# joesound212985/Deepfake-Detection-using-CLIP-Based-SigLIP-2-Vision-Transformers

Hardware: AMD Instinct MI355X
Metric: images/sec (train fwd+bwd) SigLIP-2-so400m@384 bf16 (higher is better)
Workload: dtype bf16; 1 GPU; so400m-patch14-384 encoder+pool-head train fwd+bwd, 384x384, per-GPU batch 128, seeded random weights; global_batch=128, parallelism=dp1

## Files before the change

### deepfake-detection-using-clip-based-siglip-2-vision-transformers_amd/csrc/epilogue.hip.h

```cpp
#pragma once
#include <type_traits>

#include "common.hip.h"
#include "kernels.h"

namespace sgl {

template <int NV>
__device__ __forceinline__ void epi_res_f32(float* v, const float* bias, const float* r, float* dst) {
#pragma unroll
  for (int j = 0; j < NV; ++j) v[j] = r[j] + (v[j] + bias[j]);
  Vec<float, NV>::st_nt(dst, v);
}
template <typename TOut, int NV>
__device__ __forceinline__ void epi_bias_gelu(const EpiParams& p, float* v, const float* bias, TOut* dst_u, TOut* dst_act) {
  float a[NV];
  if (p.out && p.gelu_grad_form) {
#pragma unroll
    for (int j = 0; j < NV; ++j) gelu_tanh_both(v[j] + bias[j], a[j], v[j]);
  } else {
#pragma unroll
    for (int j = 0; j < NV; ++j) {
      v[j] += bias[j];
      a[j] = gelu_tanh(v[j]);
    }
  }
  if (p.out) Vec<TOut, NV>::st_nt(dst_u, v);
  Vec<TOut, NV>::st_nt(dst_act, a);
}
__device__ __forceinline__ void qkv_split_row(int row, int tokens, int& b, int& n) {
  b = (int)((float)row * __builtin_amdgcn_rcpf((float)tokens));
  n = row - b * tokens;
  if (n < 0) { b -= 1; n += tokens; }
  else if (n >= tokens) { b += 1; n -= tokens; }
}
template <typename TOut, int NV>
__device__ __forceinline__ void epi_qkv(float* v, const float* bias, TOut* dst, int pad_chunks) {
#pragma unroll
  for (int j = 0; j < NV; ++j) v[j] += bias[j];
  Vec<TOut, NV>::st_nt(dst, v);
  if (pad_chunks) {
    float z[NV];
#pragma unroll
    for (int j = 0; j < NV; ++j) z[j] = 0.f;
    for (int k = 1; k <= pad_chunks; ++k) Vec<TOut, NV>::st_nt(dst + k * NV, z);
  }
}
template <typename TOut, int NV>
__device__ __forceinline__ void epi_gelu_bwd(const EpiParams& p, float* v, const float* u, TOut* dst) {
  if (p.gelu_grad_form) {
#pragma unroll
    for (int j = 0; j < NV; ++j) v[j] *= u[j];
  } else {
#pragma unroll
    for (int j = 0; j < NV; ++j) v[j] *= gelu_tanh_grad(u[j]);
  }
  Vec<TOut, NV>::st_nt(dst, v);
}

__device__ __forceinline__ void lds_barrier() {
  asm volatile("s_waitcnt lgkmcnt(0)" ::: "memory");
  __builtin_amdgcn_s_barrier();
  asm volatile("" ::: "memory");
}

template <int NT, int BN, int NV>
__device__ __forceinline__ void epi_colsum_fold(float* ct, const float (&csum)[NV], int t, int m0, int n0, int N,
                                                const EpiParams& p) {
  constexpr int CPR = BN / NV, GROUPS = NT / CPR;
  static_assert(NT % CPR == 0 && BN <= NT, "one fixed column set per thread, one thread per column");
  if (!p.colsum) return;
  lds_barrier();
#pragma unroll
  for (int j = 0; j < NV; ++j) ct[(t / CPR) * BN + (t % CPR) * NV + j] = csum[j];
  lds_barrier();
  if (t < BN && n0 + t < N) {
    float s = 0.f;
#pragma unroll
    for (int gI = 0; gI < GROUPS; ++gI) s += ct[gI * BN + t];
    if (p.colsum_ld > 0)
      p.colsum[(size_t)(m0 >> 7) * p.colsum_ld + n0 + t] = s;
    else
      atomicAdd(p.colsum + n0 + t, s);
  }
}

template <int EPI, typename TOut, int NV>
__device__ __forceinline__ void epi_apply(const EpiParams& p, int row, int col, int N, float* v) {
  if constexpr (EPI == EPI_STORE) {
#pragma unroll
    for (int j = 0; j < NV; ++j) v[j] *= p.alpha;
    if (p.bias) {
      float b[NV];
      Vec<float, NV>::ld(p.bias + col, b);
#pragma unroll
      for (int j = 0; j < NV; ++j) v[j] += b[j];
    }
    Vec<TOut, NV>::st_nt(reinterpret_cast<TOut*>(p.out) + (size_t)row * p.ldo + col, v);
  } else if constexpr (EPI == EPI_BIAS_GELU) {
// ... 79 lines not shown
```

### deepfake-detection-using-clip-based-siglip-2-vision-transformers_amd/csrc/gemm_bf16.hip

```cpp
#include <stdlib.h>

#include "common.hip.h"
#include "epilogue.hip.h"
#include "kernels.h"

namespace sgl {

constexpr int G_BM = 128, G_BN = 128, G_BK = 64;
constexpr int G_STAGE = (G_BM + G_BN) * G_BK * 2;
constexpr int G_CT_LD = 132;
constexpr int G_LDS = (2 * G_STAGE > G_BM * G_CT_LD * 4) ? 2 * G_STAGE : G_BM * G_CT_LD * 4;

__device__ __forceinline__ u32x4 ldg128(__amdgpu_buffer_rsrc_t r, uint32_t voff) {
  return __builtin_amdgcn_raw_buffer_load_b128(r, voff, 0, 0);
}

template <int EPI, typename TOut>
__device__ __forceinline__ void store_tile(char* smem, f32x4 (&acc)[4][4], int wr, int wc, int lane, int t, int m0,
                                           int n0, int M, int N, const EpiParams& p) {
  float* ct = reinterpret_cast<float*>(smem);
  __syncthreads();
  const int g = lane >> 4, c16 = lane & 15;
#pragma unroll
  for (int i = 0; i < 4; ++i)
// ... 197 lines not shown
  store_stage(0);
  __syncthreads();
  for (int kt = 0; kt < nk; ++kt) {
    const int cur = kt & 1;
    if (kt + 1 < nk) load_tile(kt + 1);
    const char* base = smem + cur * G_STAGE;
#pragma unroll
    for (int s = 0; s < 2; ++s) {
      const char* ba = base + s * 32 * 256 + frow;
      const char* bb = ba + OPB;
      lo_x8<TIn> af[4], bfr[4];
#pragma unroll
      for (int i = 0; i < 4; ++i) {
        const lo_x4<TIn> alo = lds_read_tr16<TIn>(ba + fa_col[i]);
        const lo_x4<TIn> ahi = lds_read_tr16<TIn>(ba + 4 * 256 + fa_col[i]);
        const lo_x4<TIn> blo = lds_read_tr16<TIn>(bb + fb_col[i]);
        const lo_x4<TIn> bhi = lds_read_tr16<TIn>(bb + 4 * 256 + fb_col[i]);
        af[i] = __builtin_shufflevector(alo, ahi, 0, 1, 2, 3, 4, 5, 6, 7);
        bfr[i] = __builtin_shufflevector(blo, bhi, 0, 1, 2, 3, 4, 5, 6, 7);
      }
#pragma unroll
      for (int i = 0; i < 4; ++i)
#pragma unroll
        for (int j = 0; j < 4; ++j)
          acc[i][j] = mfma_16x16x32(af[i], bfr[j], acc[i][j]);
    }
    if (kt + 1 < nk) store_stage(cur ^ 1);
    __syncthreads();
  }
  EpiParams pq = p;
  if (p.split_stride) pq.out = reinterpret_cast<float*>(p.out) + (size_t)blockIdx.y * p.split_stride;
  store_tile<EPI_F32, float>(smem, acc, wr, wc, lane, t, n1_0, n2_0, N1, N2, pq);
}

template <int EPI, typename TOut, typename TIn>
static hipError_t launch_nt(const TIn* A, int lda, const TIn* B, int ldb, int M, int N, int K, const EpiParams& p,
                            hipStream_t s) {
  const hipError_t e = set_max_dynamic_lds_once<&gemm_nt_kernel<EPI, TOut, TIn>>(G_LDS);
  if (e != hipSuccess) return e;
  const int tiles = ((M + G_BM - 1) / G_BM) * ((N + G_BN - 1) / G_BN);
  hipLaunchKernelGGL((gemm_nt_kernel<EPI, TOut, TIn>), dim3(tiles), dim3(256), G_LDS, s, A, lda, B, ldb, M, N, K, p);
  return hipGetLastError();
}

template <typename TIn>
static hipError_t gemm_nt_mfma(const void* A, int lda, const void* B, int ldb, int M, int N, int K, int epi,
                               int out_dtype, const EpiParams& p, hipStream_t s) {
  if (M == 0 || N == 0) return hipSuccess;
  if ((lda % 8) || (ldb % 8) || (K % 8) || K <= 0) return hipErrorInvalidValue;
  if (epi != EPI_F32 && (N % 8)) return hipErrorInvalidValue;
  if ((size_t)M * lda * 2 >= (1ull << 32) || (size_t)N * ldb * 2 >= (1ull << 32)) return hipErrorInvalidValue;
  if (M >= 2048 && N >= 256) {
    static const int tile_env = getenv("SGL_NT_TILE") ? atoi(getenv("SGL_NT_TILE")) : 0;
    const bool can384 = epi == EPI_STORE || epi == EPI_RES_F32;
    const bool pays384 = N % 192 == 0 && N % 256 != 0 && (epi == EPI_STORE || K >= 2048);
    const bool want384 = tile_env == 384 || (tile_env != 256 && pays384);
    if (can384 && want384) return gemm_nt384<TIn>(A, lda, B, ldb, M, N, K, epi, out_dtype, p, s);
    return gemm_nt256<TIn>(A, lda, B, ldb, M, N, K, epi, out_dtype, p, s);
  }
  return dispatch_epilogue<TIn>(epi, out_dtype, [&](auto tag) {
    using T = decltype(tag);
    return launch_nt<T::epi, typename T::out, TIn>((const TIn*)A, lda, (const TIn*)B, ldb, M, N, K, p, s);
  });
}
hipError_t gemm_nt_bf16(const void* A, int lda, const void* B, int ldb, int M, int N, int K, int epi, int out_dtype,
                        const EpiParams& p, hipStream_t s) {
  return gemm_nt_mfma<bf16>(A, lda, B, ldb, M, N, K, epi, out_dtype, p, s);
}
hipError_t gemm_nt_f16(const void* A, int lda, const void* B, int ldb, int M, int N, int K, int epi, int out_dtype,
                       const EpiParams& p, hipStream_t s) {
  return gemm_nt_mfma<f16>(A, lda, B, ldb, M, N, K, epi, out_dtype, p, s);
}

static bool tn_slabs_ok(const EpiParams& p, int N2, const float* split_ws) {
  return p.alpha == 1.0f && !p.bias && (N2 % 4 == 0) && (p.ldo % 4 == 0) &&
         ((((uintptr_t)p.out) | ((uintptr_t)split_ws)) & 15) == 0;
}

template <typename Launch>
static hipError_t tn_split_k(int Mred, int N1, int N2, int splits, const EpiParams& p_, hipStream_t s, float* split_ws,
                             size_t split_ws_bytes, Launch&& launch) {
  EpiParams p = p_;
  float* out = reinterpret_cast<float*>(p.out);
  if (splits < 1) splits = 1;
  int m_per = (Mred + splits - 1) / splits;
  m_per = ((m_per + G_BK - 1) / G_BK) * G_BK;
  splits = (Mred + m_per - 1) / m_per;
  if (splits > 1) {
    const size_t slab = (size_t)N1 * N2;
    if (split_ws && (size_t)splits * slab * sizeof(float) <= split_ws_bytes && tn_slabs_ok(p, N2, split_ws)) {
      EpiParams q = p;
      q.out = split_ws;
      q.ldo = N2;
      q.accumulate = 0;
      q.atomic = 0;
      q.split_stride = slab;
      const hipError_t e = launch(m_per, splits, q);
      if (e != hipSuccess) return e;
      return reduce_splits(split_ws, splits, slab, N1, N2, out, p.ldo, p.accumulate, s);
    }
    if (!p.accumulate) {
      const hipError_t e = hipMemset2DAsync(out, (size_t)p.ldo * sizeof(float), 0, (size_t)N2 * sizeof(float), N1, s);
      if (e != hipSuccess) return e;
    }
    p.atomic = 1;
  }
// ... 45 lines not shown
```

### deepfake-detection-using-clip-based-siglip-2-vision-transformers_amd/csrc/gemm_bf16_v2.hip

```cpp
#include <stdlib.h>
#ifdef SGL_TIMELINE
#include <stdio.h>
#include <string.h>
#endif

#include "common.hip.h"
#include "epilogue.hip.h"
#include "kernels.h"

namespace sgl {

constexpr int T_BK = 64;

template <int BM_, int BN_, int MI_, int MJ_>
struct NtTileShape {
  static constexpr int BM = BM_, BN = BN_, MI = MI_, MJ = MJ_;
  static constexpr int WM = 16 * MI, WN = 16 * MJ;
  static constexpr int NWR = BM / WM, NWC = BN / WN;
  static constexpr int OPA = BM * T_BK * 2;
  static constexpr int STAGE = (BM + BN) * T_BK * 2;
  static constexpr int LDS = 2 * STAGE;
  static constexpr int PA = BM / 128, PB = BN / 64, NI = 2 * PA + PB;
  static constexpr int CT_LD = BN + 4;
  static_assert(NWR * WM == BM && NWC * WN == BN && NWR * NWC == 8, "8 waves = 512 threads cover the tile");
  static_assert(MI % 2 == 0 && BM % 128 == 0 && BN % 64 == 0 && 64 % NWR == 0 && (64 / NWR) % 16 == 0, "halves, pieces, passes");
  static_assert(LDS <= 160 * 1024 && 64 * CT_LD * 4 <= LDS, "two stages, and the epilogue image, in 160 KiB of LDS");
};

struct NtTile256 : NtTileShape<256, 256, 8, 4> {
  static __device__ __forceinline__ int wr(int w) { return (w >> 1) & 1; }
  static __device__ __forceinline__ int wc(int w) { return (w & 1) + 2 * (w >> 2); }
  static __device__ __forceinline__ int b_row(int w, int q) {
    const int ul = 16 * w + 8 * (q & 1);
    return (ul >> 5) * 64 + (ul & 31) + 32 * (q >> 1);
  }
  static constexpr bool takes(int epi) { return true; }
};

struct NtTile384 : NtTileShape<384, 192, 6, 6> {
  static __device__ __forceinline__ int wr(int w) { return w & 3; }
  static __device__ __forceinline__ int wc(int w) { return w >> 2; }
  static __device__ __forceinline__ int b_row(int w, int q) { return 8 * (3 * w + q); }
  static constexpr bool takes(int epi) { return epi == EPI_STORE || epi == EPI_RES_F32 || epi == EPI_F32; }
};

constexpr int gcd_of(int a, int b) { return b == 0 ? a : gcd_of(b, a % b); }

template <typename G, int EPI, typename TOut>
__device__ __forceinline__ void store_tile_pp(char* smem, f32x4 (&acc)[G::MI][G::MJ], int wr, int wc, int lane, int t,
                                              int m0, int n0, int M, int N, const EpiParams& p) {
  static_assert(G::takes(EPI), "this tile geometry is not dispatched with this epilogue");
  float* ct = reinterpret_cast<float*>(smem);
  const int g = lane >> 4, c16 = lane & 15;
  constexpr int NV = (sizeof(TOut) == 4) ? 4 : 8;
  constexpr int CT_LD = G::CT_LD;
  constexpr int CPR = G::BN / NV;
  constexpr int WR_ROWS = 64 / G::NWR;
  constexpr int BLK = WR_ROWS / 16;
  constexpr int NPASS = G::BM / 64;
  constexpr int QN = (64 * CPR) / 512;
  constexpr int P = CPR / gcd_of(CPR, 512);
  static_assert(NPASS * BLK == G::MI && (64 * CPR) % 512 == 0 && (512 * P) % CPR == 0, "staging image and chunk walk");
  auto grow_of = [&](int pass, int row) { return m0 + (row / WR_ROWS) * G::WM + pass * WR_ROWS + row % WR_ROWS; };
  constexpr bool HAS_BIAS = (EPI == EPI_BIAS_GELU || EPI == EPI_RES_F32 || EPI == EPI_QKV);
  int tcol[P], gcol[P];
  bool col_ok[P];
  float bias[P][NV];
  size_t qkv_c0[P];
  int qkv_pad[P];
#pragma unroll
  for (int h = 0; h < P; ++h) {
    tcol[h] = ((t + 512 * h) % CPR) * NV;
    gcol[h] = n0 + tcol[h];
    col_ok[h] = gcol[h] < N;
#pragma unroll
    for (int j = 0; j < NV; ++j) bias[h][j] = 0.f;
    if constexpr (HAS_BIAS) {
      if (col_ok[h]) Vec<float, NV>::ld(p.bias + gcol[h], bias[h]);
    }
    qkv_c0[h] = 0;
    qkv_pad[h] = 0;
    if constexpr (EPI == EPI_QKV) {
      const int dm = p.heads * p.head_dim;
      const int which = gcol[h] / dm;
      const int hc = gcol[h] - which * dm;
      const int hd = hc / p.head_dim;
      const int d = hc - hd * p.head_dim;
      qkv_c0[h] = ((size_t)which * p.batch * p.heads + hd) * (size_t)p.tokens * p.head_dim_pad + d;
      qkv_pad[h] = (d + NV == p.head_dim) ? (p.head_dim_pad - p.head_dim) / NV : 0;
    }
  }
  float csum[NV];
#pragma unroll
  for (int j = 0; j < NV; ++j) csum[j] = 0.f;
  using PreT = u32x4;
  constexpr bool HAS_PRE = (EPI == EPI_RES_F32 || EPI == EPI_GELU_BWD);
// ... 41 lines not shown
        }
        continue;
      }
    }
#pragma unroll
    for (int q = 0; q < QN; ++q) {
      const int h = q % P;
      const int row = (t + 512 * q) / CPR;
      const int grow = grow_of(pass, row);
      if (grow < M && col_ok[h]) {
        float v[NV];
        Vec<float, NV>::ld(ct + row * CT_LD + tcol[h], v);
        if constexpr (EPI == EPI_RES_F32) {
          const f32x4 r = __builtin_bit_cast(f32x4, pre[pass & 1][q]);
          float rf[NV];
#pragma unroll
          for (int j = 0; j < NV; ++j) rf[j] = r[j];
          epi_res_f32<NV>(v, bias[h], rf, reinterpret_cast<float*>(p.out) + (size_t)grow * p.ldo + gcol[h]);
        } else if constexpr (EPI == EPI_BIAS_GELU) {
          epi_bias_gelu<TOut, NV>(p, v, bias[h], reinterpret_cast<TOut*>(p.out) + (size_t)grow * p.ldo + gcol[h],
                                  reinterpret_cast<TOut*>(p.out2) + (size_t)grow * p.ldo2 + gcol[h]);
        } else if constexpr (EPI == EPI_QKV) {
          int b, n;
          qkv_split_row(grow, p.tokens, b, n);
          epi_qkv<TOut, NV>(v, bias[h],
                            reinterpret_cast<TOut*>(p.out) + qkv_c0[h] + ((size_t)b * p.heads * p.tokens + n) * p.head_dim_pad,
                            qkv_pad[h]);
        } else if constexpr (EPI == EPI_GELU_BWD) {
          float u[NV];
          if constexpr (NV == 8) {
            const lo_x8<TOut> ub = __builtin_bit_cast(lo_x8<TOut>, pre[pass & 1][q]);
#pragma unroll
            for (int j = 0; j < NV; ++j) u[j] = (float)ub[j];
          } else {
            const f32x4 uf = __builtin_bit_cast(f32x4, pre[pass & 1][q]);
#pragma unroll
            for (int j = 0; j < NV; ++j) u[j] = uf[j];
          }
          epi_gelu_bwd<TOut, NV>(p, v, u, reinterpret_cast<TOut*>(p.out) + (size_t)grow * p.ldo + gcol[h]);
#pragma unroll
          for (int j = 0; j < NV; ++j) csum[j] += v[j];
        } else {
          epi_apply<EPI, TOut, NV>(p, grow, gcol[h], N, v);
        }
      }
    }
  }
  if constexpr (EPI == EPI_GELU_BWD) {
    static_assert(P == 1, "the bias-gradient fold needs one column set per thread");
    epi_colsum_fold<512, G::BN, NV>(ct, csum, t, m0, n0, N, p);
  }
}

__device__ __forceinline__ int unit_of_block(int bid, int per) { return (bid & 7) * per + (bid >> 3); }

__device__ __forceinline__ void tile_of_unit(int u, int tiles_m, int tiles_n, int& tile_m, int& tile_n, int bh = 8) {
  const int band = u / (bh * tiles_n);
  const int rows = (tiles_m - band * bh < bh) ? tiles_m - band * bh : bh;
  const int r = u - band * bh * tiles_n;
  tile_n = r / rows;
  tile_m = band * bh + (r - tile_n * rows);
}

__device__ __forceinline__ bool tile_of_local(int xcd, int v, int tiles_m, int tiles_n, int cgw, int& tm, int& tn) {
  const int r_lo = (xcd * tiles_m) >> 3, r_hi = ((xcd + 1) * tiles_m) >> 3;
  const int R = r_hi - r_lo;
  if (v >= R * tiles_n) return false;
  const int full = R * cgw;
  const int g = v / full, rem = v - g * full;
  const int w = (tiles_n - g * cgw < cgw) ? tiles_n - g * cgw : cgw;
  const int r = rem / w;
  tm = r_lo + r;
  tn = g * cgw + (rem - r * w);
  return true;
}

__device__ __forceinline__ void pp_dma16(u32x4 desc, uint32_t lds_addr, uint32_t voff) {
  asm volatile("s_mov_b32 m0, %0\n\ts_nop 0\n\tbuffer_load_dwordx4 %1, %2, 0 offen lds"
               :: "s"(lds_addr), "v"(voff), "s"(desc) : "memory");
}
__device__ __forceinline__ u32x4 pp_desc(const void* base, uint32_t bytes) {
  const uint64_t q = (uint64_t)base;
  u32x4 d = {(uint32_t)q, (uint32_t)(q >> 32) & 0xffffu, bytes, 0x00020000u};
  return d;
}
__device__ __forceinline__ u32x4 pp_desc_sgpr(u32x4 d) {
  return u32x4{(uint32_t)__builtin_amdgcn_readfirstlane((int)d[0]), (uint32_t)__builtin_amdgcn_readfirstlane((int)d[1]),
               (uint32_t)__builtin_amdgcn_readfirstlane((int)d[2]), (uint32_t)__builtin_amdgcn_readfirstlane((int)d[3])};
}
template <int NI>
__device__ __forceinline__ void pp_end_read() {
  asm volatile("s_waitcnt vmcnt(%0) lgkmcnt(0)" :: "n"(NI) : "memory");
  __builtin_amdgcn_sched_barrier(0);
  __builtin_amdgcn_s_barrier();
  __builtin_amdgcn_sched_barrier(0);
}
#define SGL_PP_END_MFMA()                 \
  do {                                    \
    __builtin_amdgcn_sched_barrier(0);    \
    __builtin_amdgcn_s_barrier();         \
    __builtin_amdgcn_sched_barrier(0);    \
  } while (0)

#ifdef SGL_TIMELINE
__device__ unsigned long long g_nt6_tl[4];
__device__ unsigned long long g_tn6_tl[12];
#define SGL_TL_STAMP(v) const unsigned long long v = __builtin_readcyclecounter()
#else
#define SGL_TL_STAMP(v)
#endif

template <typename G, int EPI, typename TOut, typename TIn>
__global__ __launch_bounds__(512, 2) void gemm_nt6_kernel(const TIn* __restrict__ A, int lda,
                                                          const TIn* __restrict__ B, int ldb, int M, int N, int K,
                                                          int tiles_m, int tiles_n, int band_h, EpiParams p) {
  extern __shared__ __attribute__((aligned(16))) char smem[];
  SGL_TL_STAMP(tl0);
  const int ntiles = tiles_m * tiles_n;
  int tile_m, tile_n;
  if (band_h < 0) {
    if (!tile_of_local(blockIdx.x & 7, blockIdx.x >> 3, tiles_m, tiles_n, -band_h, tile_m, tile_n)) return;
  } else {
    const int unit = unit_of_block(blockIdx.x, (ntiles + 7) >> 3);
    if (unit >= ntiles) return;
    tile_of_unit(unit, tiles_m, tiles_n, tile_m, tile_n, band_h);
  }
  constexpr int MI = G::MI, MJ = G::MJ, HI = MI / 2, PA = G::PA, PB = G::PB, NI = G::NI;
  const int t = threadIdx.x, lane = t & 63;
  const int w = __builtin_amdgcn_readfirstlane(t >> 6);
  const int wr = G::wr(w), wc = G::wc(w), grp = w >> 2;
  const int m0 = tile_m * G::BM, n0 = tile_n * G::BN;
  const int rows_a = (M - m0 < G::BM) ? M - m0 : G::BM;
  const int rows_b = (N - n0 < G::BN) ? N - n0 : G::BN;
  const u32x4 da = pp_desc(A + (size_t)m0 * lda, (uint32_t)(((size_t)(rows_a - 1) * lda + K) * 2));
  const u32x4 db = pp_desc(B + (size_t)n0 * ldb, (uint32_t)(((size_t)(rows_b - 1) * ldb + K) * 2));
  const uint32_t lds0 = (uint32_t)(size_t)((SGL_LDS char*)smem);

  enum { U_A0 = 0, U_B = 1, U_A1 = 2 };
  constexpr int PMAX = PA > PB ? PA : PB;
  const int drow = lane >> 3, dchunk = (lane & 7) ^ drow;
  uint32_t voff[3][PMAX], ldst[3][PMAX];
#pragma unroll
  for (int u = 0; u < 3; ++u)
#pragma unroll
    for (int q = 0; q < (u == U_B ? PB : PA); ++q) {
      const bool isA = u != U_B;
      constexpr int ppw = G::WM / 16;
      const int piece = PA * w + q;
      const int r0 = isA ? G::WM * (piece / ppw) + 8 * (piece % ppw) + (u == U_A1 ? G::WM / 2 : 0) : G::b_row(w, q);
      const int row = r0 + drow;
      voff[u][q] = (row < (isA ? rows_a : rows_b)) ? (uint32_t)(row * (isA ? lda : ldb) + dchunk * 8) * 2u : SGL_OOB;
      ldst[u][q] = lds0 + (isA ? 0 : G::OPA) + (uint32_t)r0 * 128u;
    }
  const int nk = (K + T_BK - 1) / T_BK;
  auto issue = [&](int u, int kt) {
    const int k0 = kt * T_BK;
    const bool kok = (kt < nk) && (k0 + dchunk * 8 < K);
    const uint32_t sb = (uint32_t)((kt & 1) * G::STAGE);
#pragma unroll
    for (int q = 0; q < (u == U_B ? PB : PA); ++q)
      pp_dma16(u == U_B ? db : da, ldst[u][q] + sb, (kok && voff[u][q] != SGL_OOB) ? voff[u][q] + (uint32_t)k0 * 2u : SGL_OOB);
  };

  const int frow = lane & 15, fg = lane >> 4, fsw = frow & 7;
  const uint32_t fa_base = (uint32_t)((wr * G::WM + frow) * 128);
  const uint32_t fb_base = (uint32_t)(G::OPA + (wc * G::WN + frow) * 128);
  const uint32_t c0 = (uint32_t)(((0 + fg) ^ fsw) << 4), c1 = (uint32_t)(((4 + fg) ^ fsw) << 4);
  const bool active = (n0 + wc * G::WN < N) && (m0 + wr * G::WM < M);

  f32x4 acc[MI][MJ];
#pragma unroll
  for (int i = 0; i < MI; ++i)
#pragma unroll
    for (int j = 0; j < MJ; ++j) acc[i][j] = f32x4{0.f, 0.f, 0.f, 0.f};

  issue(U_A0, 0); issue(U_B, 0); issue(U_A1, 0);
  issue(U_A0, 1); issue(U_B, 1);
  pp_end_read<NI>();
  if (grp == 1) SGL_PP_END_MFMA();

  lo_x8<TIn> fa[2 * HI], fb[2 * MJ];
  auto mfma_slot = [&](int i0) {
    if (active) {
      __builtin_amdgcn_s_setprio(1);
#pragma unroll
      for (int h = 0; h < 2; ++h)
#pragma unroll
        for (int i = 0; i < HI; ++i)
#pragma unroll
          for (int j = 0; j < MJ; ++j)
            acc[i0 + i][j] = mfma_16x16x32(fa[HI * h + i], fb[MJ * h + j], acc[i0 + i][j]);
      __builtin_amdgcn_s_setprio(0);
    }
    SGL_PP_END_MFMA();
  };
  for (int kt = 0; kt < nk; ++kt) {
    const char* base = smem + (kt & 1) * G::STAGE;
    const char* pa = base + fa_base;
    const char* pb = base + fb_base;
    if (active) {
#pragma unroll
      for (int f = 0; f < 2 * MJ; ++f) fb[f] = *reinterpret_cast<const lo_x8<TIn>*>(pb + (f % MJ) * 2048 + ((f / MJ) ? c1 : c0));
#pragma unroll
      for (int f = 0; f < 2 * HI; ++f) fa[f] = *reinterpret_cast<const lo_x8<TIn>*>(pa + (f % HI) * 2048 + ((f / HI) ? c1 : c0));
    }
    issue(U_A1, kt + 1);
    pp_end_read<NI>();
    mfma_slot(0);
    if (active) {
#pragma unroll
      for (int f = 0; f < 2 * HI; ++f) fa[f] = *reinterpret_cast<const lo_x8<TIn>*>(pa + (HI + f % HI) * 2048 + ((f / HI) ? c1 : c0));
    }
    issue(U_A0, kt + 2); issue(U_B, kt + 2);
    pp_end_read<NI>();
    mfma_slot(HI);
  }
  if (grp == 0) SGL_PP_END_MFMA();
  asm volatile("s_waitcnt vmcnt(0)" ::: "memory");
#ifdef SGL_TIMELINE
  if (p.atomic == 77) return;
#endif
  SGL_TL_STAMP(tl1);
  store_tile_pp<G, EPI, TOut>(smem, acc, wr, wc, lane, t, m0, n0, M, N, p);
#ifdef SGL_TIMELINE
  SGL_TL_STAMP(tl2);
  if (t == 0) {
    atomicAdd(&g_nt6_tl[0], tl1 - tl0);
    atomicAdd(&g_nt6_tl[1], tl2 - tl1);
    atomicAdd(&g_nt6_tl[2], 1ull);
  }
#endif
}

template <int ROWB>
__device__ __forceinline__ int tn_swz(int m) {
  static_assert(ROWB % 128 == 0, "the patterns are closed inside 256 / 128 bytes of a row");
  if constexpr (ROWB % 256 == 0) return 2 * (m & 3) + 8 * ((m >> 3) & 1);
  else return 2 * ((m >> 1) & 1) + 4 * ((m >> 3) & 1);
}

template <typename G, typename TIn>
__global__ __launch_bounds__(512, 2) void gemm_tn6_kernel(const TIn* __restrict__ A, int lda,
                                                          const TIn* __restrict__ B, int ldb, int Mred, int N1, int N2,
                                                          int m_per_split, int nsplits, int tiles_1, int tiles_2,
                                                          EpiParams p) {
  extern __shared__ __attribute__((aligned(16))) char smem[];
  constexpr int MI = G::MI, MJ = G::MJ;
  constexpr int RA = 2 * G::BM, RB = 2 * G::BN;
  constexpr int HA = G::BM / 16, HB = G::BN / 16;
  constexpr int PA = HA / 8, PB = HB / 8;
  constexpr bool BX = (HB % 8) != 0;
  constexpr int NI = 2 * PA + 2 * PB + (BX ? 1 : 0);
  static_assert(HA % 8 == 0 && (HB % 8 == 0 || HB % 8 == 4), "pieces of a k-half over 8 waves (+ one wave group)");
  const int ntiles = tiles_1 * tiles_2;
  const int nunits = ntiles * nsplits;
  const int unit = unit_of_block(blockIdx.x, (nunits + 7) >> 3);
  if (unit >= nunits) return;
  const int split = unit / ntiles, trem = unit - split * ntiles;
  const int tile1 = trem / tiles_2, tile2 = trem - tile1 * tiles_2;
  const int t = threadIdx.x, lane = t & 63;
  const int w = __builtin_amdgcn_readfirstlane(t >> 6);
  const int wr = G::wr(w), wc = G::wc(w), grp = w >> 2;
  const int n1_0 = tile1 * G::BM, n2_0 = tile2 * G::BN;
  const int m_begin = split * m_per_split;
  const int m_end = (m_begin + m_per_split < Mred) ? m_begin + m_per_split : Mred;
  const int rows = m_end - m_begin;
  const u32x4 da = pp_desc_sgpr(pp_desc(A + (size_t)m_begin * lda, (uint32_t)((size_t)rows * lda * 2)));
  const u32x4 db = pp_desc_sgpr(pp_desc(B + (size_t)m_begin * ldb, (uint32_t)((size_t)rows * ldb * 2)));
  const uint32_t lds0 = (uint32_t)(size_t)((SGL_LDS char*)smem);

  uint32_t voffA[2][PA], ldsA[2][PA], voffB[2][PB + 1], ldsB[2][PB + 1];
#pragma unroll
  for (int h = 0; h < 2; ++h) {
#pragma unroll
    for (int q = 0; q < PA; ++q) {
      const int piece = PA * w + q, pos = 1024 * piece + 16 * lane;
// ... 106 lines not shown
#undef SGL_TR6
  if (grp == 0) SGL_PP_END_MFMA();
  asm volatile("s_waitcnt vmcnt(0)" ::: "memory");
  EpiParams pq = p;
  if (p.split_stride) pq.out = reinterpret_cast<float*>(p.out) + (size_t)split * p.split_stride;
  store_tile_pp<G, EPI_F32, float>(smem, acc, wr, wc, lane, t, n1_0, n2_0, N1, N2, pq);
}

#ifdef SGL_TIMELINE
template <int NC, typename Print>
static void timeline_report(hipStream_t s, unsigned long long (&counters)[NC], Print&& print) {
  if (!getenv("SGL_TIMELINE")) return;
  unsigned long long h[NC];
  (void)hipStreamSynchronize(s);
  (void)hipMemcpyFromSymbol(h, HIP_SYMBOL(counters), sizeof(h));
  print(h);
  memset(h, 0, sizeof(h));
  (void)hipMemcpyToSymbol(HIP_SYMBOL(counters), h, sizeof(h));
}
#endif

template <typename G, int EPI, typename TOut, typename TIn>
static hipError_t launch_nt_pp(const TIn* A, int lda, const TIn* B, int ldb, int M, int N, int K, const EpiParams& p,
                               hipStream_t s) {
  const hipError_t e = set_max_dynamic_lds_once<&gemm_nt6_kernel<G, EPI, TOut, TIn>>(G::LDS);
  if (e != hipSuccess) return e;
  const int tiles_m = (M + G::BM - 1) / G::BM, tiles_n = (N + G::BN - 1) / G::BN;
  static const int band_env = getenv("SGL_BAND") ? atoi(getenv("SGL_BAND")) : 0;
  const int band_h = band_env != 0 ? band_env : -8;
  const int grid = band_h < 0 ? 8 * (((tiles_m + 7) / 8) * tiles_n)
                              : ((tiles_m * tiles_n + 7) / 8) * 8;
  EpiParams pp = p;
#ifdef SGL_TIMELINE
  static const bool skip_epi = getenv("SGL_NT6_SKIP_EPI") != nullptr;
  if (skip_epi && EPI != EPI_F32) pp.atomic = 77;
#endif
  hipLaunchKernelGGL((gemm_nt6_kernel<G, EPI, TOut, TIn>), dim3(grid), dim3(512), G::LDS, s, A, lda, B, ldb, M, N, K,
                     tiles_m, tiles_n, band_h, pp);
#ifdef SGL_TIMELINE
  timeline_report(s, g_nt6_tl, [&](const unsigned long long* h) {
    if (h[2])
      fprintf(stderr, "[timeline] gemm_nt6 %dx%d EPI %d M=%d N=%d K=%d: %llu tiles, main loop %.0f, epilogue %.0f cycles per tile\n",
              G::BM, G::BN, EPI, M, N, K, h[2], (double)h[0] / h[2], (double)h[1] / h[2]);
  });
#endif
  return hipGetLastError();
}

template <typename G, typename TIn>
static hipError_t gemm_nt_pp(const void* A, int lda, const void* B, int ldb, int M, int N, int K, int epi, int out_dtype,
                             const EpiParams& p, hipStream_t s) {
  return dispatch_epilogue<TIn>(epi, out_dtype, [&](auto tag) {
    using T = decltype(tag);
    if constexpr (G::takes(T::epi))
      return launch_nt_pp<G, T::epi, typename T::out, TIn>((const TIn*)A, lda, (const TIn*)B, ldb, M, N, K, p, s);
    else
      return hipErrorInvalidValue;
  });
}
template <typename TIn>
hipError_t gemm_nt256(const void* A, int lda, const void* B, int ldb, int M, int N, int K, int epi, int out_dtype,
                      const EpiParams& p, hipStream_t s) {
  return gemm_nt_pp<NtTile256, TIn>(A, lda, B, ldb, M, N, K, epi, out_dtype, p, s);
}
template <typename TIn>
hipError_t gemm_nt384(const void* A, int lda, const void* B, int ldb, int M, int N, int K, int epi, int out_dtype,
                      const EpiParams& p, hipStream_t s) {
  return gemm_nt_pp<NtTile384, TIn>(A, lda, B, ldb, M, N, K, epi, out_dtype, p, s);
}

template <typename G, typename TIn>
static hipError_t launch_tn_pp(const void* A, int lda, const void* B, int ldb, int Mred, int N1, int N2, int m_per,
                               int splits, const EpiParams& p, hipStream_t s) {
  const hipError_t e = set_max_dynamic_lds_once<&gemm_tn6_kernel<G, TIn>>(G::LDS);
  if (e != hipSuccess) return e;
  const int tiles_1 = (N1 + G::BM - 1) / G::BM, tiles_2 = (N2 + G::BN - 1) / G::BN;
  const int grid = ((tiles_1 * tiles_2 * splits + 7) / 8) * 8;
  hipLaunchKernelGGL((gemm_tn6_kernel<G, TIn>), dim3(grid), dim3(512), G::LDS, s, (const TIn*)A, lda, (const TIn*)B, ldb,
                     Mred, N1, N2, m_per, splits, tiles_1, tiles_2, p);
#ifdef SGL_TIMELINE
  timeline_report(s, g_tn6_tl, [&](const unsigned long long* h) {
    for (int g = 0; g < 2; ++g)
      if (h[g * 6 + 5])
        fprintf(stderr, "[timeline] gemm_tn6 %dx%d N1=%d N2=%d Mred=%d splits=%d group %d, cycles per slot pair (read slot + MFMA slot): "
                "issue reads+DMA %.0f, wait %.0f, barrier %.0f, %d MFMAs %.0f, barrier %.0f\n", G::BM, G::BN, N1, N2, Mred, splits, g,
                (double)h[g * 6 + 0] / h[g * 6 + 5], (double)h[g * 6 + 1] / h[g * 6 + 5], (double)h[g * 6 + 2] / h[g * 6 + 5],
                G::MI * G::MJ, (double)h[g * 6 + 3] / h[g * 6 + 5], (double)h[g * 6 + 4] / h[g * 6 + 5]);
  });
#endif
  return hipGetLastError();
}
template <typename TIn>
hipError_t gemm_tn256(const void* A, int lda, const void* B, int ldb, int Mred, int N1, int N2, int m_per, int splits,
                      const EpiParams& p, hipStream_t s) {
  return launch_tn_pp<NtTile256, TIn>(A, lda, B, ldb, Mred, N1, N2, m_per, splits, p, s);
}
template <typename TIn>
hipError_t gemm_tn384(const void* A, int lda, const void* B, int ldb, int Mred, int N1, int N2, int m_per, int splits,
                      const EpiParams& p, hipStream_t s) {
  return launch_tn_pp<NtTile384, TIn>(A, lda, B, ldb, Mred, N1, N2, m_per, splits, p, s);
}

#define SGL_INSTANTIATE_PP(TIn)                                                                                        \
  template hipError_t gemm_nt256<TIn>(const void*, int, const void*, int, int, int, int, int, int, const EpiParams&,   \
                                      hipStream_t);                                                                    \
  template hipError_t gemm_nt384<TIn>(const void*, int, const void*, int, int, int, int, int, int, const EpiParams&,   \
                                      hipStream_t);                                                                    \
  template hipError_t gemm_tn256<TIn>(const void*, int, const void*, int, int, int, int, int, int, const EpiParams&,   \
                                      hipStream_t);                                                                    \
  template hipError_t gemm_tn384<TIn>(const void*, int, const void*, int, int, int, int, int, int, const EpiParams&,   \
                                      hipStream_t);
SGL_INSTANTIATE_PP(bf16)
SGL_INSTANTIATE_PP(f16)
#undef SGL_INSTANTIATE_PP

}
```

### deepfake-detection-using-clip-based-siglip-2-vision-transformers_amd/csrc/kernels.h

```cpp
#pragma once
#include <hip/hip_runtime.h>
#include <stddef.h>
#include <stdint.h>

#include "siglip_hip.h"

namespace sgl {

enum DType : int {
  DT_F32 = 0,
  DT_BF16 = 1,
  DT_F32_MFMA = 2,
  DT_F16 = 3,
};
static inline size_t dtype_size(int dt) { return (dt == DT_BF16 || dt == DT_F16) ? 2 : 4; }

template <auto Kernel>
hipError_t set_max_dynamic_lds_once(int bytes) {
  static bool done = false;
  if (done) return hipSuccess;
  const hipError_t e =
      hipFuncSetAttribute(reinterpret_cast<const void*>(Kernel), hipFuncAttributeMaxDynamicSharedMemorySize, bytes);
  done = e == hipSuccess;
  return e;
// ... 67 lines not shown
  int nmat = 0, nvec = 0, ntiles = 0;
};
void cast_job_add(CastJob& job, const float* src, int R, int C, int lds_, void* dst, int Rp, int Cp, int ldd, void* dst_t,
                  int ldt);
void cast_job_add_vec(CastJob& job, const float* src, int n, float* dst, int np);
hipError_t cast_job_run(const CastJob& job, int dst_dtype, hipStream_t s);
hipError_t split3_rows(const float* src, int R, int C, int ld, void* dst, int Cs, int b_side, hipStream_t s);
hipError_t split3_stack(const float* src, int R, int C, int ld, void* dst, int Cs, int b_side, hipStream_t s);
int colsum_chunks(int M);
hipError_t colsum(const void* in, int dtype, int ld, int M, int N, int n_out, float* partial ,
                  float* out, int accumulate, hipStream_t s);
hipError_t batch_sum(const float* in, int B, size_t n, float* out, int accumulate, hipStream_t s);
hipError_t vecmat_f32(const float* v, const float* W, int rows, int cols, float* scratch, float* out, int accumulate,
                      hipStream_t s);
hipError_t pos_resize(const float* table, int g0, float* out, int gh, int gw, int D, hipStream_t s);
hipError_t pos_resize_bwd(const float* dout, int gh, int gw, float* dtable, int g0, int D, hipStream_t s);
hipError_t copy_f32(const float* src, float* dst, size_t n, hipStream_t s);
hipError_t cast_f32(const float* src, void* dst, int dst_dtype, size_t n, hipStream_t s);
hipError_t add_f32(const float* a, const float* b, float* out, size_t n, hipStream_t s);
hipError_t zero_unless_nonfinite(const float* src, float* dst, int n, int accumulate, hipStream_t s);

static inline size_t pool_attn_lds_floats(int N, int DP, int backward) {
  const size_t part = (size_t)N * (DP / 8) > (size_t)256 * 8 ? (size_t)N * (DP / 8) : (size_t)256 * 8;
  return part + (backward ? 2 : 1) * (size_t)N + 8;
}
static inline int pool_attn_max_tokens(int DP, int backward) {
  return (int)((64 * 1024 / sizeof(float) - 8) / (size_t)(DP / 8 + (backward ? 2 : 1)));
}
hipError_t pool_attn_fwd(const float* q, const void* K, const void* V, int dtype, void* out ,
                         float* probs , int B, int H, int N, int dh, int DP, hipStream_t s);
hipError_t pool_attn_bwd(const float* q, const void* K, const void* V, int dtype, const float* probs,
                         const float* dout , void* dkv ,
                         float* dq_partial , int B, int H, int N, int dh, int DP, hipStream_t s);

hipError_t gemm_f32_generic(const float* A, long sam, long sak, const float* B, long sbn, long sbk, int M, int N,
                            int K, int epi, int out_dtype, const EpiParams& p, hipStream_t s);

hipError_t gemm_nt_bf16(const void* A, int lda, const void* B, int ldb, int M, int N, int K, int epi,
                        int out_dtype, const EpiParams& p, hipStream_t s);
hipError_t reduce_splits(const float* ws, int splits, size_t stride, int N1, int N2, float* out, int ldo, int accumulate,
                         hipStream_t s);
hipError_t gemm_tn_bf16(const void* A, int lda, const void* B, int ldb, int Mred, int N1, int N2, int splits,
                        const EpiParams& p, hipStream_t s, float* split_ws = nullptr, size_t split_ws_bytes = 0);
hipError_t gemm_nt_f16(const void* A, int lda, const void* B, int ldb, int M, int N, int K, int epi, int out_dtype,
                       const EpiParams& p, hipStream_t s);
hipError_t gemm_tn_f16(const void* A, int lda, const void* B, int ldb, int Mred, int N1, int N2, int splits,
                       const EpiParams& p, hipStream_t s, float* split_ws = nullptr, size_t split_ws_bytes = 0);
template <typename TIn>
hipError_t gemm_nt256(const void* A, int lda, const void* B, int ldb, int M, int N, int K, int epi, int out_dtype,
                      const EpiParams& p, hipStream_t s);
template <typename TIn>
hipError_t gemm_nt384(const void* A, int lda, const void* B, int ldb, int M, int N, int K, int epi, int out_dtype,
                      const EpiParams& p, hipStream_t s);
template <typename TIn>
hipError_t gemm_tn256(const void* A, int lda, const void* B, int ldb, int Mred, int N1, int N2, int m_per, int splits,
                      const EpiParams& p, hipStream_t s);
template <typename TIn>
hipError_t gemm_tn384(const void* A, int lda, const void* B, int ldb, int Mred, int N1, int N2, int m_per, int splits,
                      const EpiParams& p, hipStream_t s);

struct TnPlan {
  int tile, splits, m_per;
};
constexpr TnPlan tn_plan(int Mred, int N1, int N2, size_t ws_bytes, int tile = 0) {
  TnPlan best = {0, 0, 0};
  long best_cost = 0;
  for (int g = 0; g < 2; ++g) {
    const int bm = g ? 384 : 256, bn = g ? 192 : 256, area8 = g ? 9 : 8;
    if (tile != 0 && tile != bm) continue;
    const int tiles = ((N1 + bm - 1) / bm) * ((N2 + bn - 1) / bn);
    for (int sp = 1; sp == 1 || (tiles * sp <= 256 && Mred / sp >= 1024); ++sp) {
      if (sp > 1 && (size_t)sp * N1 * N2 * sizeof(float) > ws_bytes) break;
      const int m_per = ((Mred + sp - 1) / sp + 63) / 64 * 64;
      const long cost = (long)area8 * m_per;
      if (best.tile == 0 || cost < best_cost) {
        best = {bm, (Mred + m_per - 1) / m_per, m_per};
        best_cost = cost;
      }
    }
  }
  return best;
}
constexpr bool tn_plan_is(int Mred, int N1, int N2, size_t ws_bytes, int tile, int splits) {
  const TnPlan p = tn_plan(Mred, N1, N2, ws_bytes);
  return (tile == 0 || p.tile == tile) && p.splits == splits;
}
constexpr size_t kTnSlabBytes = (size_t)256 * 384 * 192 * 4;
static_assert(tn_plan_is(93312, 1152, 1152, kTnSlabBytes, 384, 14), "out_proj dW");
static_assert(tn_plan_is(93312, 3456, 1152, kTnSlabBytes, 384, 4), "QKV dW");
static_assert(tn_plan_is(93312, 4304, 1152, kTnSlabBytes, 256, 3), "fc1 dW");
static_assert(tn_plan_is(93312, 1152, 4304, kTnSlabBytes, 256, 3), "fc2 dW");
static_assert(tn_plan_is(4133, 520, 1152, kTnSlabBytes, 0, 4) && tn_plan(4133, 520, 1152, kTnSlabBytes).m_per == 1088, "digest case");
static_assert(tn_plan_is(2048, 512, 512, kTnSlabBytes, 256, 2) && tn_plan(2048, 512, 512, kTnSlabBytes).m_per == 1024, "digest case");

hipError_t attn_fwd(const void* q, const void* k, const void* v, int dtype, void* out, float* lse, int B, int H,
                    int N, int dh, int DP, int ld_qkv, hipStream_t s);
hipError_t attn_bwd(const void* q, const void* k, const void* v, const void* out, const void* dout,
                    const float* lse, int dtype, void* dqkv, float* delta, int B, int H, int N, int dh, int DP,
                    int ld_qkv, hipStream_t s);

bool attn_probs_shape_ok(int dtype, int B, int H, int N, int dh, int DP);
hipError_t attn_probs(const void* q, const void* k, const float* lse, float* out, int dtype, int B, int H, int N, int dh,
                      int DP, int mode, hipStream_t s);
hipError_t probs_head_mean(const float* probs, float* out, int B, int H, int N, hipStream_t s);

bool attn_grad_probs_shape_ok(int dtype, int B, int H, int N, int dh, int DP);
// ... 7 lines not shown
```

Baseline: 442.9 images/sec.

## Add 256x288 QKV GEMM tile with whole-head LDS-staged padded epilogue

```diff
diff --git a/deepfake-detection-using-clip-based-siglip-2-vision-transformers_amd/csrc/epilogue.hip.h b/deepfake-detection-using-clip-based-siglip-2-vision-transformers_amd/csrc/epilogue.hip.h
--- a/deepfake-detection-using-clip-based-siglip-2-vision-transformers_amd/csrc/epilogue.hip.h
+++ b/deepfake-detection-using-clip-based-siglip-2-vision-transformers_amd/csrc/epilogue.hip.h
@@ -45,6 +45,21 @@
     for (int j = 0; j < NV; ++j) z[j] = 0.f;
     for (int k = 1; k <= pad_chunks; ++k) Vec<TOut, NV>::st_nt(dst + k * NV, z);
   }
+}
+template <typename TOut>
+__device__ __forceinline__ void epi_qkv_halves(f32x4 first, f32x4 second, bool swapped, bool pad, TOut* dst) {
+  static_assert(sizeof(TOut) == 2, "16-bit outputs: eight columns are one 16-byte chunk");
+  lo_x4<TOut> pf, ps;
+#pragma unroll
+  for (int j = 0; j < 4; ++j) {
+    pf[j] = (TOut)first[j];
+    ps[j] = (TOut)second[j];
+  }
+  const u32x2 uf = __builtin_bit_cast(u32x2, pf), us = __builtin_bit_cast(u32x2, ps);
+  const u32x2 lo = swapped ? us : uf, hi = swapped ? uf : us;
+  u32x4 o = {lo[0], lo[1], hi[0], hi[1]};
+  if (pad) o = u32x4{0u, 0u, 0u, 0u};
+  __builtin_nontemporal_store(o, reinterpret_cast<u32x4*>(dst));
 }
 template <typename TOut, int NV>
 __device__ __forceinline__ void epi_gelu_bwd(const EpiParams& p, float* v, const float* u, TOut* dst) {
diff --git a/deepfake-detection-using-clip-based-siglip-2-vision-transformers_amd/csrc/gemm_bf16.hip b/deepfake-detection-using-clip-based-siglip-2-vision-transformers_amd/csrc/gemm_bf16.hip
--- a/deepfake-detection-using-clip-based-siglip-2-vision-transformers_amd/csrc/gemm_bf16.hip
+++ b/deepfake-detection-using-clip-based-siglip-2-vision-transformers_amd/csrc/gemm_bf16.hip
@@ -273,6 +273,11 @@
   if ((size_t)M * lda * 2 >= (1ull << 32) || (size_t)N * ldb * 2 >= (1ull << 32)) return hipErrorInvalidValue;
   if (M >= 2048 && N >= 256) {
     static const int tile_env = getenv("SGL_NT_TILE") ? atoi(getenv("SGL_NT_TILE")) : 0;
+    if (epi == EPI_QKV && out_dtype == (std::is_same<TIn, f16>::value ? DT_F16 : DT_BF16)) {
+      const bool can288 = nt288_takes_qkv(N, p);
+      if (tile_env == 288 && !can288) return hipErrorInvalidValue;
+      if (can288 && (tile_env == 288 || tile_env == 0)) return gemm_nt288<TIn>(A, lda, B, ldb, M, N, K, epi, out_dtype, p, s);
+    }
     const bool can384 = epi == EPI_STORE || epi == EPI_RES_F32;
     const bool pays384 = N % 192 == 0 && N % 256 != 0 && (epi == EPI_STORE || K >= 2048);
     const bool want384 = tile_env == 384 || (tile_env != 256 && pays384);
diff --git a/deepfake-detection-using-clip-based-siglip-2-vision-transformers_amd/csrc/gemm_bf16_v2.hip b/deepfake-detection-using-clip-based-siglip-2-vision-transformers_amd/csrc/gemm_bf16_v2.hip
--- a/deepfake-detection-using-clip-based-siglip-2-vision-transformers_amd/csrc/gemm_bf16_v2.hip
+++ b/deepfake-detection-using-clip-based-siglip-2-vision-transformers_amd/csrc/gemm_bf16_v2.hip
@@ -12,18 +12,30 @@
 
 constexpr int T_BK = 64;
 
-template <int BM_, int BN_, int MI_, int MJ_>
+template <int BM_, int BN_, int MI_, int MJ_, bool SPLIT_B_ = false, int CT_LD_ = BN_ + 4, int QKV_HD_ = 0, int QKV_HDP_ = 0>
 struct NtTileShape {
   static constexpr int BM = BM_, BN = BN_, MI = MI_, MJ = MJ_;
   static constexpr int WM = 16 * MI, WN = 16 * MJ;
   static constexpr int NWR = BM / WM, NWC = BN / WN;
+  static constexpr int BNI = (BN + 63) / 64 * 64;
   static constexpr int OPA = BM * T_BK * 2;
-  static constexpr int STAGE = (BM + BN) * T_BK * 2;
+  static constexpr int STAGE = (BM + BNI) * T_BK * 2;
   static constexpr int LDS = 2 * STAGE;
-  static constexpr int PA = BM / 128, PB = BN / 64, NI = 2 * PA + PB;
-  static constexpr int CT_LD = BN + 4;
+  static constexpr bool SPLIT_B = SPLIT_B_;
+  static constexpr int J0 = (MJ + 1) / 2, J1 = MJ - J0;
+  static constexpr int P0 = SPLIT_B ? BM / 64 : BM / 128;
+  static constexpr int P1 = SPLIT_B ? (NWC * J0 * 16 + BNI - BN) / 64 : BNI / 64;
+  static constexpr int P2 = SPLIT_B ? (NWC * J1 * 16) / 64 : BM / 128;
+  static constexpr int NI = P0 + P1 + P2;
+  static constexpr int CT_LD = CT_LD_;
+  static constexpr int QKV_HD = QKV_HD_, QKV_HDP = QKV_HDP_;
   static_assert(NWR * WM == BM && NWC * WN == BN && NWR * NWC == 8, "8 waves = 512 threads cover the tile");
-  static_assert(MI % 2 == 0 && BM % 128 == 0 && BN % 64 == 0 && 64 % NWR == 0 && (64 / NWR) % 16 == 0, "halves, pieces, passes");
+  static_assert(BM % 128 == 0 && 64 % NWR == 0 && (64 / NWR) % 16 == 0, "pieces, passes");
+  static_assert(SPLIT_B ? ((NWC * J0 * 16 + BNI - BN) % 64 == 0 && (NWC * J1 * 16) % 64 == 0 && (J0 * 16) % 8 == 0)
+                        : (MI % 2 == 0 && BN % 64 == 0), "every wave issues the same number of pieces of every unit");
+  static_assert(QKV_HD == 0 || (BN % QKV_HD == 0 && QKV_HD % 8 == 0 && QKV_HDP % 8 == 0 && QKV_HDP >= QKV_HD &&
+                                (64 * (BN / QKV_HD) * (QKV_HDP / 8)) % 512 == 0), "whole heads, whole chunk rounds");
+  static_assert(CT_LD >= BN && CT_LD % 4 == 0, "16-byte aligned staging rows");
   static_assert(LDS <= 160 * 1024 && 64 * CT_LD * 4 <= LDS, "two stages, and the epilogue image, in 160 KiB of LDS");
 };
 
@@ -42,6 +54,20 @@
   static __device__ __forceinline__ int wc(int w) { return w >> 2; }
   static __device__ __forceinline__ int b_row(int w, int q) { return 8 * (3 * w + q); }
   static constexpr bool takes(int epi) { return epi == EPI_STORE || epi == EPI_RES_F32 || epi == EPI_F32; }
+};
+
+struct NtTile288 : NtTileShape<256, 288, 4, 9, true, 336, 72, 80> {
+  static __device__ __forceinline__ int wr(int w) { return w & 3; }
+  static __device__ __forceinline__ int wc(int w) { return w >> 2; }
+  static __device__ __forceinline__ int b_row(int w, int half, int q) {
+    if (half == 0) {
+      const int piece = P1 * w + q;
+      return piece < NWC * 2 * J0 ? WN * (piece / (2 * J0)) + 8 * (piece % (2 * J0)) : BN + 8 * (piece - NWC * 2 * J0);
+    }
+    const int piece = P2 * w + q;
+    return WN * (piece / (2 * J1)) + 16 * J0 + 8 * (piece % (2 * J1));
+  }
+  static constexpr bool takes(int epi) { return epi == EPI_QKV; }
 };
 
 constexpr int gcd_of(int a, int b) { return b == 0 ? a : gcd_of(b, a % b); }
@@ -189,6 +215,56 @@
   }
 }
 
+template <typename G, typename TOut>
+__device__ __forceinline__ void store_tile_qkv_heads(char* smem, f32x4 (&acc)[G::MI][G::MJ], int wr, int wc, int lane,
+                                                     int t, int m0, int n0, int M, const EpiParams& p) {
+  static_assert(G::takes(EPI_QKV) && G::QKV_HD > 0, "this tile geometry does not hold whole heads");
+  float* ct = reinterpret_cast<float*>(smem);
+  const int g = lane >> 4, c16 = lane & 15;
+  constexpr int NV = 8, CT_LD = G::CT_LD;
+  constexpr int HPT = G::BN / G::QKV_HD;
+  constexpr int CPH = G::QKV_HDP / NV;
+  constexpr int DCH = G::QKV_HD / NV;
+  constexpr int CHD = 64 * CPH;
+  constexpr int QN = (HPT * CHD) / 512;
+  constexpr int WR_ROWS = 64 / G::NWR, BLK = WR_ROWS / 16, NPASS = G::BM / 64;
+  static_assert(NPASS * BLK == G::MI, "staging image");
+  float bias[G::MJ];
+#pragma unroll
+  for (int j = 0; j < G::MJ; ++j) bias[j] = p.bias[n0 + wc * G::WN + j * 16 + c16];
+  const int gh0 = n0 / G::QKV_HD, which = gh0 / p.heads;
+  const int rows0 = (which * p.batch * p.heads + (gh0 - which * p.heads)) * p.tokens;
+  const bool swapped = (lane >> 3) & 1;
+#pragma unroll
+  for (int pass = 0; pass < NPASS; ++pass) {
+    lds_barrier();
+#pragma unroll
+    for (int i2 = 0; i2 < BLK; ++i2)
+#pragma unroll
+      for (int j = 0; j < G::MJ; ++j)
+#pragma unroll
+        for (int r = 0; r < 4; ++r)
+          ct[(wr * WR_ROWS + i2 * 16 + g * 4 + r) * CT_LD + wc * G::WN + j * 16 + c16] = acc[BLK * pass + i2][j][r] + bias[j];
+    lds_barrier();
+#pragma unroll
+    for (int q = 0; q < QN; ++q) {
+      const int i = t + 512 * q;
+      const int head = i / CHD, rem = i % CHD, row = rem / CPH, c = rem % CPH;
+      const int grow = m0 + (row / WR_ROWS) * G::WM + pass * WR_ROWS + row % WR_ROWS;
+      if (grow < M) {
+        const float* src = ct + row * CT_LD + head * G::QKV_HD + NV * (c < DCH ? c : DCH - 1);
+        const f32x4 first = *reinterpret_cast<const f32x4*>(src + (swapped ? 4 : 0));
+        const f32x4 second = *reinterpret_cast<const f32x4*>(src + (swapped ? 0 : 4));
+        int b, n;
+        qkv_split_row(grow, p.tokens, b, n);
+        const int drow = rows0 + (b * p.heads + head) * p.tokens + n;
+        epi_qkv_halves<TOut>(first, second, swapped, c >= DCH,
+                             reinterpret_cast<TOut*>(p.out) + (size_t)drow * G::QKV_HDP + NV * c);
+      }
+    }
+  }
+}
+
 __device__ __forceinline__ int unit_of_block(int bid, int per) { return (bid & 7) * per + (bid >> 3); }
 
 __device__ __forceinline__ void tile_of_unit(int u, int tiles_m, int tiles_n, int& tile_m, int& tile_n, int bh = 8) {
@@ -262,7 +338,8 @@
     if (unit >= ntiles) return;
     tile_of_unit(unit, tiles_m, tiles_n, tile_m, tile_n, band_h);
   }
-  constexpr int MI = G::MI, MJ = G::MJ, HI = MI / 2, PA = G::PA, PB = G::PB, NI = G::NI;
+  constexpr int MI = G::MI, MJ = G::MJ, HI = MI / 2, J0 = G::J0, J1 = G::J1, NI = G::NI;
+  constexpr bool SB = G::SPLIT_B;
   const int t = threadIdx.x, lane = t & 63;
   const int w = __builtin_amdgcn_readfirstlane(t >> 6);
   const int wr = G::wr(w), wc = G::wc(w), grp = w >> 2;
@@ -273,18 +350,23 @@
   const u32x4 db = pp_desc(B + (size_t)n0 * ldb, (uint32_t)(((size_t)(rows_b - 1) * ldb + K) * 2));
   const uint32_t lds0 = (uint32_t)(size_t)((SGL_LDS char*)smem);
 
-  enum { U_A0 = 0, U_B = 1, U_A1 = 2 };
-  constexpr int PMAX = PA > PB ? PA : PB;
+  constexpr int PU[3] = {G::P0, G::P1, G::P2};
+  constexpr int PMAX = G::P0 > G::P1 ? (G::P0 > G::P2 ? G::P0 : G::P2) : (G::P1 > G::P2 ? G::P1 : G::P2);
   const int drow = lane >> 3, dchunk = (lane & 7) ^ drow;
   uint32_t voff[3][PMAX], ldst[3][PMAX];
 #pragma unroll
   for (int u = 0; u < 3; ++u)
 #pragma unroll
-    for (int q = 0; q < (u == U_B ? PB : PA); ++q) {
-      const bool isA = u != U_B;
-      constexpr int ppw = G::WM / 16;
-      const int piece = PA * w + q;
-      const int r0 = isA ? G::WM * (piece / ppw) + 8 * (piece % ppw) + (u == U_A1 ? G::WM / 2 : 0) : G::b_row(w, q);
+    for (int q = 0; q < PU[u]; ++q) {
+      const bool isA = SB ? u == 0 : u != 1;
+      int r0;
+      if constexpr (SB) {
+        r0 = isA ? 8 * (G::P0 * w + q) : G::b_row(w, u - 1, q);
+      } else {
+        constexpr int ppw = G::WM / 16;
+        const int piece = G::P0 * w + q;
+        r0 = isA ? G::WM * (piece / ppw) + 8 * (piece % ppw) + (u == 2 ? G::WM / 2 : 0) : G::b_row(w, q);
+      }
       const int row = r0 + drow;
       voff[u][q] = (row < (isA ? rows_a : rows_b)) ? (uint32_t)(row * (isA ? lda : ldb) + dchunk * 8) * 2u : SGL_OOB;
       ldst[u][q] = lds0 + (isA ? 0 : G::OPA) + (uint32_t)r0 * 128u;
@@ -294,9 +376,10 @@
     const int k0 = kt * T_BK;
     const bool kok = (kt < nk) && (k0 + dchunk * 8 < K);
     const uint32_t sb = (uint32_t)((kt & 1) * G::STAGE);
-#pragma unroll
-    for (int q = 0; q < (u == U_B ? PB : PA); ++q)
-      pp_dma16(u == U_B ? db : da, ldst[u][q] + sb, (kok && voff[u][q] != SGL_OOB) ? voff[u][q] + (uint32_t)k0 * 2u : SGL_OOB);
+    const bool isA = SB ? u == 0 : u != 1;
+#pragma unroll
+    for (int q = 0; q < PU[u]; ++q)
+      pp_dma16(isA ? da : db, ldst[u][q] + sb, (kok && voff[u][q] != SGL_OOB) ? voff[u][q] + (uint32_t)k0 * 2u : SGL_OOB);
   };
 
   const int frow = lane & 15, fg = lane >> 4, fsw = frow & 7;
@@ -311,22 +394,26 @@
 #pragma unroll
     for (int j = 0; j < MJ; ++j) acc[i][j] = f32x4{0.f, 0.f, 0.f, 0.f};
 
-  issue(U_A0, 0); issue(U_B, 0); issue(U_A1, 0);
-  issue(U_A0, 1); issue(U_B, 1);
+  issue(0, 0); issue(1, 0); issue(2, 0);
+  issue(0, 1); issue(1, 1);
   pp_end_read<NI>();
   if (grp == 1) SGL_PP_END_MFMA();
 
-  lo_x8<TIn> fa[2 * HI], fb[2 * MJ];
-  auto mfma_slot = [&](int i0) {
+  constexpr int NA = SB ? MI : HI, NB = SB ? J0 : MJ;
+  lo_x8<TIn> fa[2 * NA], fb[2 * NB];
+  auto mfma_slot = [&](auto half) {
+    constexpr int hf = decltype(half)::value;
+    constexpr int i0 = SB ? 0 : hf * HI, ni = SB ? MI : HI;
+    constexpr int j0 = SB ? hf * J0 : 0, nj = SB ? (hf ? J1 : J0) : MJ;
     if (active) {
       __builtin_amdgcn_s_setprio(1);
 #pragma unroll
       for (int h = 0; h < 2; ++h)
 #pragma unroll
-        for (int i = 0; i < HI; ++i)
-#pragma unroll
-          for (int j = 0; j < MJ; ++j)
-            acc[i0 + i][j] = mfma_16x16x32(fa[HI * h + i], fb[MJ * h + j], acc[i0 + i][j]);
+        for (int i = 0; i < ni; ++i)
+#pragma unroll
+          for (int j = 0; j < nj; ++j)
+            acc[i0 + i][j0 + j] = mfma_16x16x32(fa[ni * h + i], fb[nj * h + j], acc[i0 + i][j0 + j]);
       __builtin_amdgcn_s_setprio(0);
     }
     SGL_PP_END_MFMA();
@@ -337,20 +424,25 @@
     const char* pb = base + fb_base;
     if (active) {
 #pragma unroll
-      for (int f = 0; f < 2 * MJ; ++f) fb[f] = *reinterpret_cast<const lo_x8<TIn>*>(pb + (f % MJ) * 2048 + ((f / MJ) ? c1 : c0));
-#pragma unroll
-      for (int f = 0; f < 2 * HI; ++f) fa[f] = *reinterpret_cast<const lo_x8<TIn>*>(pa + (f % HI) * 2048 + ((f / HI) ? c1 : c0));
-    }
-    issue(U_A1, kt + 1);
+      for (int f = 0; f < 2 * NB; ++f) fb[f] = *reinterpret_cast<const lo_x8<TIn>*>(pb + (f % NB) * 2048 + ((f / NB) ? c1 : c0));
+#pragma unroll
+      for (int f = 0; f < 2 * NA; ++f) fa[f] = *reinterpret_cast<const lo_x8<TIn>*>(pa + (f % NA) * 2048 + ((f / NA) ? c1 : c0));
+    }
+    issue(2, kt + 1);
     pp_end_read<NI>();
-    mfma_slot(0);
+    mfma_slot(std::integral_constant<int, 0>{});
     if (active) {
-#pragma unroll
-      for (int f = 0; f < 2 * HI; ++f) fa[f] = *reinterpret_cast<const lo_x8<TIn>*>(pa + (HI + f % HI) * 2048 + ((f / HI) ? c1 : c0));
-    }
-    issue(U_A0, kt + 2); issue(U_B, kt + 2);
+      if constexpr (SB) {
+#pragma unroll
+        for (int f = 0; f < 2 * J1; ++f) fb[f] = *reinterpret_cast<const lo_x8<TIn>*>(pb + (J0 + f % J1) * 2048 + ((f / J1) ? c1 : c0));
+      } else {
+#pragma unroll
+        for (int f = 0; f < 2 * HI; ++f) fa[f] = *reinterpret_cast<const lo_x8<TIn>*>(pa + (HI + f % HI) * 2048 + ((f / HI) ? c1 : c0));
+      }
+    }
+    issue(0, kt + 2); issue(1, kt + 2);
     pp_end_read<NI>();
-    mfma_slot(HI);
+    mfma_slot(std::integral_constant<int, 1>{});
   }
   if (grp == 0) SGL_PP_END_MFMA();
   asm volatile("s_waitcnt vmcnt(0)" ::: "memory");
@@ -358,7 +450,10 @@
   if (p.atomic == 77) return;
 #endif
   SGL_TL_STAMP(tl1);
-  store_tile_pp<G, EPI, TOut>(smem, acc, wr, wc, lane, t, m0, n0, M, N, p);
+  if constexpr (EPI == EPI_QKV && G::QKV_HD > 0)
+    store_tile_qkv_heads<G, TOut>(smem, acc, wr, wc, lane, t, m0, n0, M, p);
+  else
+    store_tile_pp<G, EPI, TOut>(smem, acc, wr, wc, lane, t, m0, n0, M, N, p);
 #ifdef SGL_TIMELINE
   SGL_TL_STAMP(tl2);
   if (t == 0) {
@@ -571,7 +666,7 @@
                              const EpiParams& p, hipStream_t s) {
   return dispatch_epilogue<TIn>(epi, out_dtype, [&](auto tag) {
     using T = decltype(tag);
-    if constexpr (G::takes(T::epi))
+    if constexpr (G::takes(T::epi) && (G::QKV_HD == 0 || sizeof(typename T::out) == 2))
       return launch_nt_pp<G, T::epi, typename T::out, TIn>((const TIn*)A, lda, (const TIn*)B, ldb, M, N, K, p, s);
     else
       return hipErrorInvalidValue;
@@ -586,6 +681,13 @@
 hipError_t gemm_nt384(const void* A, int lda, const void* B, int ldb, int M, int N, int K, int epi, int out_dtype,
                       const EpiParams& p, hipStream_t s) {
   return gemm_nt_pp<NtTile384, TIn>(A, lda, B, ldb, M, N, K, epi, out_dtype, p, s);
+}
+static_assert(NtTile288::QKV_HD == NT288_HEAD_DIM && NtTile288::QKV_HDP == NT288_HEAD_DIM_PAD && NtTile288::BN == NT288_BN, "kernels.h");
+template <typename TIn>
+hipError_t gemm_nt288(const void* A, int lda, const void* B, int ldb, int M, int N, int K, int epi, int out_dtype,
+                      const EpiParams& p, hipStream_t s) {
+  if (epi != EPI_QKV || !nt288_takes_qkv(N, p)) return hipErrorInvalidValue;
+  return gemm_nt_pp<NtTile288, TIn>(A, lda, B, ldb, M, N, K, epi, out_dtype, p, s);
 }
 
 template <typename G, typename TIn>
@@ -625,6 +727,8 @@
                                       hipStream_t);                                                                    \
   template hipError_t gemm_nt384<TIn>(const void*, int, const void*, int, int, int, int, int, int, const EpiParams&,   \
                                       hipStream_t);                                                                    \
+  template hipError_t gemm_nt288<TIn>(const void*, int, const void*, int, int, int, int, int, int, const EpiParams&,   \
+                                      hipStream_t);                                                                    \
   template hipError_t gemm_tn256<TIn>(const void*, int, const void*, int, int, int, int, int, int, const EpiParams&,   \
                                       hipStream_t);                                                                    \
   template hipError_t gemm_tn384<TIn>(const void*, int, const void*, int, int, int, int, int, int, const EpiParams&,   \
diff --git a/deepfake-detection-using-clip-based-siglip-2-vision-transformers_amd/csrc/kernels.h b/deepfake-detection-using-clip-based-siglip-2-vision-transformers_amd/csrc/kernels.h
--- a/deepfake-detection-using-clip-based-siglip-2-vision-transformers_amd/csrc/kernels.h
+++ b/deepfake-detection-using-clip-based-siglip-2-vision-transformers_amd/csrc/kernels.h
@@ -143,6 +143,14 @@
 template <typename TIn>
 hipError_t gemm_nt384(const void* A, int lda, const void* B, int ldb, int M, int N, int K, int epi, int out_dtype,
                       const EpiParams& p, hipStream_t s);
+constexpr int NT288_BN = 288, NT288_HEAD_DIM = 72, NT288_HEAD_DIM_PAD = 80;
+inline bool nt288_takes_qkv(int N, const EpiParams& p) {
+  return p.head_dim == NT288_HEAD_DIM && p.head_dim_pad == NT288_HEAD_DIM_PAD && p.heads > 0 &&
+         N == 3 * p.heads * NT288_HEAD_DIM && N % NT288_BN == 0;
+}
+template <typename TIn>
+hipError_t gemm_nt288(const void* A, int lda, const void* B, int ldb, int M, int N, int K, int epi, int out_dtype,
+                      const EpiParams& p, hipStream_t s);
 template <typename TIn>
 hipError_t gemm_tn256(const void* A, int lda, const void* B, int ldb, int Mred, int N1, int N2, int m_per, int splits,
                       const EpiParams& p, hipStream_t s);
```

Measured after the change: 448.3 images/sec, median of 6. +1.2%, better.
